# PKU-DAIR/Hetu-Galvatron

Measured on NVIDIA H100. Metric: tokens/sec Llama-3.2-1B-shaped ZeRO-2 training step at 1/2/4/8 H100 vs ref CPU, higher is better.
Workload: dtype bf16

## Files before the change

hetu-galvatron_b200/csrc/bg_gemm.cu:

```cuda
#include <stdlib.h>

#include "bg_ctx.cuh"

using namespace bg;

namespace {

constexpr int BLOCK_M = 128, BLOCK_N = 128, BLOCK_K = 64, WGMMA_K = 16;
constexpr int WIDE_N = 256;
constexpr int kABytes = BLOCK_M * BLOCK_K * 2;
constexpr int kStoreCols = 64;
constexpr int kStoreBytes = BLOCK_M * kStoreCols * 2;
constexpr int kEpiThreads = 256, kThreads = kEpiThreads + 32;
constexpr int kProducerWarp = kEpiThreads / 32;
constexpr int kWgOffset = 8192;
constexpr int kGroupM = 16;

template <int kBlockN>
struct Tile {
    static constexpr bool kWide = kBlockN == WIDE_N;
    static constexpr int kStages = kWide ? 4 : 5;
    static constexpr int kNumStoreBufs = kWide ? 1 : 2;
    static constexpr int kMaxRegs = kWide ? 168 : 136;
    static constexpr int kSlimCtas = kWide ? 2 : 3;
// ... 28 lines not shown
}
__device__ __forceinline__ void mbar_expect_tx(uint32_t bar, uint32_t bytes) {
    asm volatile("mbarrier.arrive.expect_tx.shared::cta.b64 _, [%0], %1;" ::"r"(bar), "r"(bytes) : "memory");
}
__device__ __forceinline__ void tma_load_2d(uint32_t dst, const CUtensorMap* map, uint32_t bar, int c0, int c1) {
    asm volatile("cp.async.bulk.tensor.2d.shared::cluster.global.mbarrier::complete_tx::bytes [%0], [%1, {%3, %4}], [%2];"
                 ::"r"(dst), "l"(map), "r"(bar), "r"(c0), "r"(c1) : "memory");
}
__device__ __forceinline__ void tma_store_2d(const CUtensorMap* map, uint32_t src, int c0, int c1) {
    asm volatile("cp.async.bulk.tensor.2d.global.shared::cta.bulk_group [%0, {%2, %3}], [%1];"
                 ::"l"(map), "r"(src), "r"(c0), "r"(c1) : "memory");
}
__device__ __forceinline__ void tma_store_commit() { asm volatile("cp.async.bulk.commit_group;" ::: "memory"); }
template <int N>
__device__ __forceinline__ void tma_store_wait_read() { asm volatile("cp.async.bulk.wait_group.read %0;" ::"n"(N) : "memory"); }
template <int N>
__device__ __forceinline__ void tma_store_wait_all() { asm volatile("cp.async.bulk.wait_group %0;" ::"n"(N) : "memory"); }
__device__ __forceinline__ void fence_proxy_async() { asm volatile("fence.proxy.async.shared::cta;" ::: "memory"); }
__device__ __forceinline__ void epi_bar_sync() { asm volatile("bar.sync 1, %0;" ::"n"(kEpiThreads) : "memory"); }
__device__ __forceinline__ bool elect_one() {
    uint32_t pred;
    asm volatile("{\n\t.reg .pred p;\n\telect.sync _|p, 0xffffffff;\n\tselp.u32 %0, 1, 0, p;\n\t}" : "=r"(pred));
    return pred != 0;
}

__device__ __forceinline__ void wgmma_fence() { asm volatile("wgmma.fence.sync.aligned;" ::: "memory"); }
__device__ __forceinline__ void wgmma_commit() { asm volatile("wgmma.commit_group.sync.aligned;" ::: "memory"); }
template <int N>
__device__ __forceinline__ void wgmma_wait() { asm volatile("wgmma.wait_group.sync.aligned %0;" ::"n"(N) : "memory"); }
template <int kNumAcc>
__device__ __forceinline__ void fence_acc(float* d) {
#pragma unroll
    for (int i = 0; i < kNumAcc; ++i) asm volatile("" : "+f"(d[i])::"memory");
}

template <int kTransA, int kTransB>
__device__ __forceinline__ void wgmma_m64n128(float* d, uint64_t desc_a, uint64_t desc_b, uint32_t accumulate) {
    asm volatile(
        "{\n\t.reg .pred p;\n\t"
        "setp.ne.b32 p, %66, 0;\n\t"
        "wgmma.mma_async.sync.aligned.m64n128k16.f32.bf16.bf16 "
        "{%0, %1, %2, %3, %4, %5, %6, %7, %8, %9, %10, %11, %12, %13, %14, %15, "
        "%16, %17, %18, %19, %20, %21, %22, %23, %24, %25, %26, %27, %28, %29, %30, %31, "
        "%32, %33, %34, %35, %36, %37, %38, %39, %40, %41, %42, %43, %44, %45, %46, %47, "
        "%48, %49, %50, %51, %52, %53, %54, %55, %56, %57, %58, %59, %60, %61, %62, %63}, "
        "%64, %65, p, 1, 1, %67, %68;\n\t}"
        : "+f"(d[0]), "+f"(d[1]), "+f"(d[2]), "+f"(d[3]), "+f"(d[4]), "+f"(d[5]), "+f"(d[6]), "+f"(d[7]),
          "+f"(d[8]), "+f"(d[9]), "+f"(d[10]), "+f"(d[11]), "+f"(d[12]), "+f"(d[13]), "+f"(d[14]), "+f"(d[15]),
          "+f"(d[16]), "+f"(d[17]), "+f"(d[18]), "+f"(d[19]), "+f"(d[20]), "+f"(d[21]), "+f"(d[22]), "+f"(d[23]),
          "+f"(d[24]), "+f"(d[25]), "+f"(d[26]), "+f"(d[27]), "+f"(d[28]), "+f"(d[29]), "+f"(d[30]), "+f"(d[31]),
          "+f"(d[32]), "+f"(d[33]), "+f"(d[34]), "+f"(d[35]), "+f"(d[36]), "+f"(d[37]), "+f"(d[38]), "+f"(d[39]),
          "+f"(d[40]), "+f"(d[41]), "+f"(d[42]), "+f"(d[43]), "+f"(d[44]), "+f"(d[45]), "+f"(d[46]), "+f"(d[47]),
          "+f"(d[48]), "+f"(d[49]), "+f"(d[50]), "+f"(d[51]), "+f"(d[52]), "+f"(d[53]), "+f"(d[54]), "+f"(d[55]),
          "+f"(d[56]), "+f"(d[57]), "+f"(d[58]), "+f"(d[59]), "+f"(d[60]), "+f"(d[61]), "+f"(d[62]), "+f"(d[63])
        : "l"(desc_a), "l"(desc_b), "r"(accumulate), "n"(kTransA), "n"(kTransB));
}

template <int kTransA, int kTransB>
__device__ __forceinline__ void wgmma_m64n256(float* d, uint64_t desc_a, uint64_t desc_b, uint32_t accumulate) {
    asm volatile(
        "{\n\t.reg .pred p;\n\t"
        "setp.ne.b32 p, %130, 0;\n\t"
        "wgmma.mma_async.sync.aligned.m64n256k16.f32.bf16.bf16 "
        "{%0, %1, %2, %3, %4, %5, %6, %7, %8, %9, %10, %11, %12, %13, %14, %15, "
        "%16, %17, %18, %19, %20, %21, %22, %23, %24, %25, %26, %27, %28, %29, %30, %31, "
        "%32, %33, %34, %35, %36, %37, %38, %39, %40, %41, %42, %43, %44, %45, %46, %47, "
// ... 9 lines not shown
          "+f"(d[24]), "+f"(d[25]), "+f"(d[26]), "+f"(d[27]), "+f"(d[28]), "+f"(d[29]), "+f"(d[30]), "+f"(d[31]),
          "+f"(d[32]), "+f"(d[33]), "+f"(d[34]), "+f"(d[35]), "+f"(d[36]), "+f"(d[37]), "+f"(d[38]), "+f"(d[39]),
          "+f"(d[40]), "+f"(d[41]), "+f"(d[42]), "+f"(d[43]), "+f"(d[44]), "+f"(d[45]), "+f"(d[46]), "+f"(d[47]),
          "+f"(d[48]), "+f"(d[49]), "+f"(d[50]), "+f"(d[51]), "+f"(d[52]), "+f"(d[53]), "+f"(d[54]), "+f"(d[55]),
          "+f"(d[56]), "+f"(d[57]), "+f"(d[58]), "+f"(d[59]), "+f"(d[60]), "+f"(d[61]), "+f"(d[62]), "+f"(d[63]),
          "+f"(d[64]), "+f"(d[65]), "+f"(d[66]), "+f"(d[67]), "+f"(d[68]), "+f"(d[69]), "+f"(d[70]), "+f"(d[71]),
          "+f"(d[72]), "+f"(d[73]), "+f"(d[74]), "+f"(d[75]), "+f"(d[76]), "+f"(d[77]), "+f"(d[78]), "+f"(d[79]),
          "+f"(d[80]), "+f"(d[81]), "+f"(d[82]), "+f"(d[83]), "+f"(d[84]), "+f"(d[85]), "+f"(d[86]), "+f"(d[87]),
          "+f"(d[88]), "+f"(d[89]), "+f"(d[90]), "+f"(d[91]), "+f"(d[92]), "+f"(d[93]), "+f"(d[94]), "+f"(d[95]),
          "+f"(d[96]), "+f"(d[97]), "+f"(d[98]), "+f"(d[99]), "+f"(d[100]), "+f"(d[101]), "+f"(d[102]), "+f"(d[103]),
          "+f"(d[104]), "+f"(d[105]), "+f"(d[106]), "+f"(d[107]), "+f"(d[108]), "+f"(d[109]), "+f"(d[110]), "+f"(d[111]),
          "+f"(d[112]), "+f"(d[113]), "+f"(d[114]), "+f"(d[115]), "+f"(d[116]), "+f"(d[117]), "+f"(d[118]), "+f"(d[119]),
          "+f"(d[120]), "+f"(d[121]), "+f"(d[122]), "+f"(d[123]), "+f"(d[124]), "+f"(d[125]), "+f"(d[126]), "+f"(d[127])
        : "l"(desc_a), "l"(desc_b), "r"(accumulate), "n"(kTransA), "n"(kTransB));
}

__device__ __forceinline__ uint64_t make_smem_desc(uint32_t smem_addr, uint32_t lbo_bytes, uint32_t sbo_bytes) {
    uint64_t d = 0;
    d |= (uint64_t)((smem_addr >> 4) & 0x3fff);
    d |= (uint64_t)((lbo_bytes >> 4) & 0x3fff) << 16;
    d |= (uint64_t)((sbo_bytes >> 4) & 0x3fff) << 32;
    d |= (uint64_t)1 << 62;
    return d;
}

struct TileCoord { int m, n; };
enum { kPlain = 0, kScatterMode = 1, kGatherMode = 2 };

template <int kMode>
struct FuseParams {};

template <>
struct FuseParams<kPlain> {
    int group_m;
};

__device__ __forceinline__ TileCoord tile_of_virtual(int t, int m_blocks, int n_blocks, int group_m) {
    const int per_group = group_m * n_blocks;
    const int g = t / per_group, first_m = g * group_m;
    const int rows = min(group_m, m_blocks - first_m);
    const int r = t - g * per_group;
    return {first_m + r % rows, r / rows};
}

template <>
struct FuseParams<kScatterMode> {
    CUtensorMap dst[BG_MAX_PEERS];
    uint32_t* flags[BG_MAX_PEERS];
    int p, me, rows_per_rank;
};

template <>
struct FuseParams<kGatherMode> {
    CUtensorMap a_local;
    const uint32_t* flags;
    uint32_t target;
    int p, me, blocks_per_rank;
    unsigned long long timeout_ns;
    int* err;
};

template <int kMode>
__device__ __forceinline__ int map_m(int mv, int m_blocks, const FuseParams<kMode>& fp) {
    if constexpr (kMode == kScatterMode) {
        int m = mv + ((fp.me + 1) % fp.p) * (fp.rows_per_rank / BLOCK_M);
        return m >= m_blocks ? m - m_blocks : m;
    } else if constexpr (kMode == kGatherMode) {
        const int c = mv / fp.p, k = mv - c * fp.p;
        int slot = fp.me + k; if (slot >= fp.p) slot -= fp.p;
        return slot * fp.blocks_per_rank + c;
    } else {
        return mv;
    }
}
template <int kMode>
__device__ __forceinline__ TileCoord tile_of(int t, int m_blocks, int n_blocks, const FuseParams<kMode>& fp) {
    int group_m = kGroupM;
    if constexpr (kMode == kPlain) group_m = fp.group_m;
    TileCoord tc = tile_of_virtual(t, m_blocks, n_blocks, group_m);
    tc.m = map_m<kMode>(tc.m, m_blocks, fp);
    return tc;
}

template <int kLayout, int kMode = kPlain, int kBlockN = BLOCK_N>
__global__ void __maxnreg__(Tile<kBlockN>::kMaxRegs) gemm_bf16_kernel(const __grid_constant__ CUtensorMap map_a,
                                                                const __grid_constant__ CUtensorMap map_b,
                                                                const __grid_constant__ CUtensorMap map_c,
                                                                const __nv_bfloat16* __restrict__ c_old, int M, int N, int K,
                                                                int accumulate,
                                                                const __grid_constant__ FuseParams<kMode> sp) {
    static_assert(kMode == kPlain || kBlockN == BLOCK_N, "the fused modes wait on peers: they keep the three-slim-CTA tile");
    constexpr bool kScatter = kMode == kScatterMode, kGather = kMode == kGatherMode;
    constexpr bool kAMn = kLayout == kNT, kBMn = kLayout != kTN;
    constexpr int kStages = Tile<kBlockN>::kStages, kStageBytes = Tile<kBlockN>::kStageBytes;
    constexpr int kNumStoreBufs = Tile<kBlockN>::kNumStoreBufs;
    extern __shared__ uint8_t smem_raw[];
    uint8_t* smem = reinterpret_cast<uint8_t*>((reinterpret_cast<uintptr_t>(smem_raw) + 1023) & ~uintptr_t(1023));
    uint8_t* smem_store = smem + kStages * kStageBytes;
    uint64_t* bars = reinterpret_cast<uint64_t*>(smem_store + kNumStoreBufs * kStoreBytes);
    uint64_t* full_bar = bars;
    uint64_t* empty_bar = bars + kStages;

    const int warp = threadIdx.x >> 5, lane = threadIdx.x & 31;
    const int m_blocks = (M + BLOCK_M - 1) / BLOCK_M, n_blocks = (N + kBlockN - 1) / kBlockN;
    const int num_tiles = m_blocks * n_blocks, k_blocks = (K + BLOCK_K - 1) / BLOCK_K;

    if constexpr (kScatter) {
        asm volatile("griddepcontrol.launch_dependents;" ::: "memory");
    }
    if (warp == kProducerWarp && lane == 0) {
        asm volatile("prefetch.tensormap [%0];" ::"l"(&map_a) : "memory");
        asm volatile("prefetch.tensormap [%0];" ::"l"(&map_b) : "memory");
        asm volatile("prefetch.tensormap [%0];" ::"l"(&map_c) : "memory");
        for (int i = 0; i < kStages; ++i) { mbar_init(smem_u32(full_bar + i), 1); mbar_init(smem_u32(empty_bar + i), kEpiThreads / 32); }
        asm volatile("fence.mbarrier_init.release.cluster;" ::: "memory");
    }
    __syncthreads();

    if (warp == kProducerWarp) {
        if (elect_one()) {
            int stage = 0; uint32_t phase = 0;
            for (int t = blockIdx.x; t < num_tiles; t += gridDim.x) {
                const TileCoord tc = tile_of<kMode>(t, m_blocks, n_blocks, sp);
                const CUtensorMap* amap = &map_a;
                int a_row = tc.m * BLOCK_M;
                if constexpr (kGather) {
                    const int slot = tc.m / sp.blocks_per_rank, c = tc.m - slot * sp.blocks_per_rank;
                    if (slot == sp.me) {
                        amap = &sp.a_local; a_row = c * BLOCK_M;
                    } else {
                        const uint32_t* f = sp.flags + slot * sp.blocks_per_rank + c;
                        unsigned long long t0 = 0; unsigned spins = 0;
                        while (true) {
                            uint32_t v;
                            asm volatile("ld.acquire.sys.global.u32 %0, [%1];" : "=r"(v) : "l"(f) : "memory");
                            if (v >= sp.target) break;
                            if ((++spins & 0x3ff) == 0) {
                                unsigned long long now = gtimer();
                                if (t0 == 0) t0 = now;
                                else if (now - t0 > sp.timeout_ns) {
                                    if (atomicCAS(sp.err + 1, 0, 4) == 0) { sp.err[2] = (int)blockIdx.x; sp.err[3] = tc.m; sp.err[4] = (int)v; sp.err[5] = (int)sp.target; sp.err[6] = slot; }
                                    *sp.err = BG_ETIMEOUT; __threadfence_system(); __trap();
                                }
                            }
                        }
                        asm volatile("fence.proxy.async.global;" ::: "memory");
                    }
// ... 2 lines not shown
                    mbar_wait(smem_u32(empty_bar + stage), phase ^ 1);
                    const uint32_t bar = smem_u32(full_bar + stage);
                    const uint32_t sa = smem_u32(smem + stage * kStageBytes), sb = sa + kABytes;
                    mbar_expect_tx(bar, kStageBytes);
                    if (kAMn) {
#pragma unroll
                        for (int j = 0; j < BLOCK_M / 64; ++j) tma_load_2d(sa + j * (BLOCK_K * 128), &map_a, bar, tc.m * BLOCK_M + j * 64, kb * BLOCK_K);
                    } else {
                        tma_load_2d(sa, amap, bar, kb * BLOCK_K, a_row);
                    }
                    if (kBMn) {
#pragma unroll
                        for (int j = 0; j < kBlockN / 64; ++j) tma_load_2d(sb + j * (BLOCK_K * 128), &map_b, bar, tc.n * kBlockN + j * 64, kb * BLOCK_K);
                    } else {
                        tma_load_2d(sb, &map_b, bar, kb * BLOCK_K, tc.n * kBlockN);
                    }
                    if (++stage == kStages) { stage = 0; phase ^= 1; }
                }
            }
        }
    } else {
        const int wg = warp >> 2;
        const int frag_row = wg * 64 + (warp & 3) * 16 + (lane >> 2);
        const int frag_col = (lane & 3) * 2;
        const bool issuer = threadIdx.x == 0;
        constexpr uint32_t a_lbo = kAMn ? BLOCK_K * 128 : 0, b_lbo = kBMn ? BLOCK_K * 128 : 0;
        constexpr uint32_t a_kstep = kAMn ? WGMMA_K * 128 : WGMMA_K * 2, b_kstep = kBMn ? WGMMA_K * 128 : WGMMA_K * 2;
        float acc[kBlockN / 2];
#pragma unroll
        for (int i = 0; i < kBlockN / 2; ++i) acc[i] = 0.f;
        int stage = 0; uint32_t phase = 0;
        int buf = 0;
        uint32_t* prev_flag = nullptr;
        for (int t = blockIdx.x; t < num_tiles; t += gridDim.x) {
            const TileCoord tc = tile_of<kMode>(t, m_blocks, n_blocks, sp);
            int prev_stage = 0;
            for (int kb = 0; kb < k_blocks; ++kb) {
                mbar_wait(smem_u32(full_bar + stage), phase);
                const uint32_t sa = smem_u32(smem + stage * kStageBytes) + wg * kWgOffset;
                const uint32_t sb = smem_u32(smem + stage * kStageBytes) + kABytes;
                wgmma_fence();
#pragma unroll
                for (int k = 0; k < BLOCK_K / WGMMA_K; ++k) {
                    const uint64_t da = make_smem_desc(sa + k * a_kstep, a_lbo, 1024);
                    const uint64_t db = make_smem_desc(sb + k * b_kstep, b_lbo, 1024);
                    if constexpr (kBlockN == WIDE_N) wgmma_m64n256<kAMn ? 1 : 0, kBMn ? 1 : 0>(acc, da, db, (kb | k) != 0);
                    else wgmma_m64n128<kAMn ? 1 : 0, kBMn ? 1 : 0>(acc, da, db, (kb | k) != 0);
                }
                wgmma_commit();
                wgmma_wait<1>();
                if (kb > 0 && lane == 0) mbar_arrive(smem_u32(empty_bar + prev_stage));
                prev_stage = stage;
                if (++stage == kStages) { stage = 0; phase ^= 1; }
            }
            wgmma_wait<0>();
            fence_acc<kBlockN / 2>(acc);
            if (lane == 0) mbar_arrive(smem_u32(empty_bar + prev_stage));
#pragma unroll
            for (int c = 0; c < kBlockN / kStoreCols; ++c) {
                const int n0 = tc.n * kBlockN + c * kStoreCols;
                if (n0 >= N) break;
                float* v = acc + c * (kStoreCols / 2);
                if (accumulate && Tile<kBlockN>::kWide) {
#pragma unroll
                    for (int h = 0; h < 2; ++h) {
                        const int grow = tc.m * BLOCK_M + frag_row + 8 * h;
                        if (grow < M) {
                            const uint32_t* src = reinterpret_cast<const uint32_t*>(c_old + (long long)grow * N + n0 + frag_col);
#pragma unroll
                            for (int j = 0; j < 8; ++j) {
                                if (n0 + j * 8 < N) {
                                    const float2 o = bf2_to_f2(src[j * 4]);
                                    v[j * 4 + 2 * h] += o.x;
                                    v[j * 4 + 2 * h + 1] += o.y;
                                }
                            }
                        }
                    }
                } else if (accumulate) {
#pragma unroll
                    for (int h = 0; h < 2; ++h) {
                        const long long grow = (long long)tc.m * BLOCK_M + frag_row + 8 * h;
                        if (grow < M) {
#pragma unroll
                            for (int j = 0; j < 8; ++j) {
                                if (n0 + j * 8 < N) {
                                    const float2 o = bf2_to_f2(*reinterpret_cast<const uint32_t*>(c_old + grow * N + n0 + j * 8 + frag_col));
                                    v[j * 4 + 2 * h] += o.x;
                                    v[j * 4 + 2 * h + 1] += o.y;
                                }
                            }
                        }
                    }
                }
                if (issuer) tma_store_wait_read<kNumStoreBufs - 1>();
                epi_bar_sync();
                uint8_t* sbuf = smem_store + buf * kStoreBytes;
                if constexpr (Tile<kBlockN>::kWide) {
                    uint32_t srow = smem_u32(sbuf) + frag_row * 128 + ((frag_row & 7) << 4) + frag_col * 2;
                    asm volatile("" : "+r"(srow));
#pragma unroll
                    for (int h = 0; h < 2; ++h) {
#pragma unroll
                        for (int j = 0; j < 8; ++j)
                            asm volatile("st.shared.u32 [%0], %1;" ::"r"((srow + h * 1024) ^ (j << 4)),
                                         "r"(f2_to_bf2(v[j * 4 + 2 * h], v[j * 4 + 2 * h + 1])) : "memory");
                    }
                } else {
#pragma unroll
                    for (int h = 0; h < 2; ++h) {
                        const int row = frag_row + 8 * h;
#pragma unroll
                        for (int j = 0; j < 8; ++j)
                            *reinterpret_cast<uint32_t*>(sbuf + row * 128 + ((j ^ (row & 7)) << 4) + frag_col * 2) =
                                f2_to_bf2(v[j * 4 + 2 * h], v[j * 4 + 2 * h + 1]);
                    }
                }
                fence_proxy_async();
                epi_bar_sync();
                if (issuer) {
                    if constexpr (kScatter) {
                        const int row0 = tc.m * BLOCK_M, owner = row0 / sp.rows_per_rank;
                        tma_store_2d(&sp.dst[owner], smem_u32(sbuf), n0, sp.me * sp.rows_per_rank + (row0 - owner * sp.rows_per_rank));
                    } else {
                        tma_store_2d(&map_c, smem_u32(sbuf), n0, tc.m * BLOCK_M);
                    }
                    tma_store_commit();
                }
                if constexpr (kNumStoreBufs > 1) buf ^= 1;
            }
            if constexpr (kScatter) {
                if (issuer) {
                    if (prev_flag != nullptr) {
                        asm volatile("cp.async.bulk.wait_group %0;" ::"n"(kBlockN / kStoreCols) : "memory");
                        __threadfence_system();
                        asm volatile("red.release.sys.global.add.u32 [%0], 1;" ::"l"(prev_flag) : "memory");
                    }
                    const int row0 = tc.m * BLOCK_M, owner = row0 / sp.rows_per_rank;
                    prev_flag = sp.flags[owner] + ((row0 - owner * sp.rows_per_rank) / BLOCK_M) * n_blocks + tc.n;
                }
            }
        }
        if (issuer) {
            tma_store_wait_all<0>();
            if constexpr (kScatter) {
                if (prev_flag != nullptr) {
                    __threadfence_system();
                    asm volatile("red.release.sys.global.add.u32 [%0], 1;" ::"l"(prev_flag) : "memory");
                }
            }
        }
    }
}

typedef CUresult (*EncodeTiledFn)(CUtensorMap*, CUtensorMapDataType, cuuint32_t, void*, const cuuint64_t*, const cuuint64_t*,
                                  const cuuint32_t*, const cuuint32_t*, CUtensorMapInterleave, CUtensorMapSwizzle,
                                  CUtensorMapL2promotion, CUtensorMapFloatOOBfill);

EncodeTiledFn encode_fn() {
    static EncodeTiledFn fn = nullptr;
    static std::once_flag once;
    std::call_once(once, [] {
        void* p = nullptr;
        cudaDriverEntryPointQueryResult q;
        if (cudaGetDriverEntryPoint("cuTensorMapEncodeTiled", &p, cudaEnableDefault, &q) == cudaSuccess && q == cudaDriverEntryPointSuccess)
            fn = (EncodeTiledFn)p;
    });
    return fn;
}

int make_map(CUtensorMap* map, const void* ptr, long long rows, long long cols, int box_cols, int box_rows) {
    EncodeTiledFn fn = encode_fn();
    if (!fn) return fail(BG_ECUDA, "cuTensorMapEncodeTiled entry point not available");
    cuuint64_t dims[2] = {(cuuint64_t)cols, (cuuint64_t)rows};
    cuuint64_t strides[1] = {(cuuint64_t)cols * 2};
    cuuint32_t box[2] = {(cuuint32_t)box_cols, (cuuint32_t)box_rows};
    cuuint32_t estr[2] = {1, 1};
    CUresult r = fn(map, CU_TENSOR_MAP_DATA_TYPE_BFLOAT16, 2, const_cast<void*>(ptr), dims, strides, box, estr,
                    CU_TENSOR_MAP_INTERLEAVE_NONE, CU_TENSOR_MAP_SWIZZLE_128B, CU_TENSOR_MAP_L2_PROMOTION_L2_256B,
                    CU_TENSOR_MAP_FLOAT_OOB_FILL_NONE);
    if (r == CUDA_ERROR_INVALID_CONTEXT) {
        cudaFree(0);
        r = fn(map, CU_TENSOR_MAP_DATA_TYPE_BFLOAT16, 2, const_cast<void*>(ptr), dims, strides, box, estr,
               CU_TENSOR_MAP_INTERLEAVE_NONE, CU_TENSOR_MAP_SWIZZLE_128B, CU_TENSOR_MAP_L2_PROMOTION_L2_256B,
               CU_TENSOR_MAP_FLOAT_OOB_FILL_NONE);
    }
    if (r != CUDA_SUCCESS) return fail(BG_ECUDA, "cuTensorMapEncodeTiled failed (%d) rows=%lld cols=%lld", (int)r, rows, cols);
    return BG_OK;
}

int g_num_sms = 0;

}

int bg_preload_gemm();

static int gemm_setup() {
    if (g_num_sms == 0) {
        int dev = 0;
        BG_CUDA(cudaGetDevice(&dev));
        int sms = 0;
        BG_CUDA(cudaDeviceGetAttribute(&sms, cudaDevAttrMultiProcessorCount, dev));
#define BG_SMEM(K, W) BG_CUDA(cudaFuncSetAttribute(K, cudaFuncAttributeMaxDynamicSharedMemorySize, Tile<W>::kSmemBytes))
        BG_SMEM(gemm_bf16_kernel<kTN>, BLOCK_N); BG_SMEM(gemm_bf16_kernel<kNN>, BLOCK_N); BG_SMEM(gemm_bf16_kernel<kNT>, BLOCK_N);
        BG_SMEM((gemm_bf16_kernel<kTN, kPlain, WIDE_N>), WIDE_N); BG_SMEM((gemm_bf16_kernel<kNN, kPlain, WIDE_N>), WIDE_N);
        BG_SMEM((gemm_bf16_kernel<kNT, kPlain, WIDE_N>), WIDE_N);
        BG_SMEM((gemm_bf16_kernel<kTN, kScatterMode>), BLOCK_N); BG_SMEM((gemm_bf16_kernel<kNN, kScatterMode>), BLOCK_N);
        BG_SMEM((gemm_bf16_kernel<kNT, kScatterMode>), BLOCK_N);
        BG_SMEM((gemm_bf16_kernel<kTN, kGatherMode>), BLOCK_N); BG_SMEM((gemm_bf16_kernel<kNN, kGatherMode>), BLOCK_N);
#undef BG_SMEM
        g_num_sms = sms;
    }
    return BG_OK;
}



static int make_ab_maps(CUtensorMap* ma, CUtensorMap* mb, const void* a, const void* b, long long m, long long n, long long k, int layout,
                        int block_n = BLOCK_N) {
    int rc = layout == kNT ? make_map(ma, a, k, m, 64, BLOCK_K) : make_map(ma, a, m, k, BLOCK_K, BLOCK_M);
    if (rc) return rc;
    return layout == kTN ? make_map(mb, b, n, k, BLOCK_K, block_n) : make_map(mb, b, k, n, 64, BLOCK_K);
}

static int gemm_launch(const void* a, const void* b, void* c, const void* addend, long long m, long long n, long long k, int layout, void* stream);

extern "C" int bg_gemm_bf16(const void* a, const void* b, void* c, long long m, long long n, long long k, int layout,
                            int accumulate, void* stream) {
    return gemm_launch(a, b, c, accumulate ? c : nullptr, m, n, k, layout, stream);
}

extern "C" int bg_gemm_bf16_add(const void* a, const void* b, void* c, const void* addend, long long m, long long n, long long k,
                                int layout, void* stream) {
    if (addend == nullptr || (uintptr_t)addend % 16) return fail(BG_EINVAL, "bg_gemm_bf16_add: addend must be a 16-B aligned [M][N] bf16 tensor");
    return gemm_launch(a, b, c, addend, m, n, k, layout, stream);
}

template <int kBlockN>
static int plain_launch(const void* a, const void* b, void* c, const void* addend, long long m, long long n, long long k, int layout, void* stream);

static int gemm_launch(const void* a, const void* b, void* c, const void* addend, long long m, long long n, long long k, int layout, void* stream) {
    if (layout < 0 || layout > 2) return fail(BG_EINVAL, "bg_gemm_bf16: layout %d", layout);
    if (m <= 0 || n <= 0 || k <= 0 || m % 8 || n % 8 || k % 8)
        return fail(BG_EINVAL, "bg_gemm_bf16: m,n,k (%lld,%lld,%lld) must be positive multiples of 8", m, n, k);
    if (((uintptr_t)a | (uintptr_t)b | (uintptr_t)c) % 16) return fail(BG_EINVAL, "bg_gemm_bf16: pointers must be 16-B aligned");
    return n > BLOCK_N ? plain_launch<WIDE_N>(a, b, c, addend, m, n, k, layout, stream)
                       : plain_launch<BLOCK_N>(a, b, c, addend, m, n, k, layout, stream);
}

template <int kBlockN>
static int plain_launch(const void* a, const void* b, void* c, const void* addend, long long m, long long n, long long k, int layout, void* stream) {
    CUtensorMap ma, mb, mc;
    int rc = make_ab_maps(&ma, &mb, a, b, m, n, k, layout, kBlockN);
    if (rc) return rc;
    rc = make_map(&mc, c, m, n, kStoreCols, BLOCK_M);
    if (rc) return rc;
    rc = gemm_setup();
    if (rc) return rc;
    const long long n_blocks = (n + kBlockN - 1) / kBlockN, tiles = ((m + BLOCK_M - 1) / BLOCK_M) * n_blocks;
    const int grid = (int)(tiles < g_num_sms ? tiles : g_num_sms);
    cudaStream_t st = (cudaStream_t)stream;
    const __nv_bfloat16* c_old = (const __nv_bfloat16*)addend;
    const int accumulate = addend != nullptr;
    constexpr int smem = Tile<kBlockN>::kSmemBytes;
    FuseParams<kPlain> plain;
    plain.group_m = n_blocks <= 16 ? 4 : 16;
    if (layout == kTN) gemm_bf16_kernel<kTN, kPlain, kBlockN><<<grid, kThreads, smem, st>>>(ma, mb, mc, c_old, (int)m, (int)n, (int)k, accumulate, plain);
    else if (layout == kNN) gemm_bf16_kernel<kNN, kPlain, kBlockN><<<grid, kThreads, smem, st>>>(ma, mb, mc, c_old, (int)m, (int)n, (int)k, accumulate, plain);
    else gemm_bf16_kernel<kNT, kPlain, kBlockN><<<grid, kThreads, smem, st>>>(ma, mb, mc, c_old, (int)m, (int)n, (int)k, accumulate, plain);
    BG_CHECK_LAUNCH();
    return BG_OK;
}

namespace {

struct Bcast {
    char* out[BG_MAX_PEERS];
    char* mc;
    int on;
};

__device__ __forceinline__ void mm_st_16g(void* mc, const uint4& v) {
    asm volatile("multimem.st.relaxed.sys.global.v4.f32 [%0], {%1,%2,%3,%4};" ::"l"(mc), "f"(__uint_as_float(v.x)),
                 "f"(__uint_as_float(v.y)), "f"(__uint_as_float(v.z)), "f"(__uint_as_float(v.w)) : "memory");
}

__global__ void __launch_bounds__(128, 8) tile_reduce_kernel(const __nv_bfloat16* __restrict__ partial, uint32_t* __restrict__ flags,
                                                          __nv_bfloat16* __restrict__ out, int p, int me, int rows_per_rank, int N,
                                                          int n_blocks, int local_tiles, const __grid_constant__ Bcast bc,
                                                          unsigned long long timeout_ns, int* err) {
    for (int lt = blockIdx.x; lt < local_tiles; lt += gridDim.x) {
        if (threadIdx.x == 0) {
            unsigned long long t0 = 0;
            unsigned spins = 0;
            while (true) {
                uint32_t v;
                asm volatile("ld.acquire.sys.global.u32 %0, [%1];" : "=r"(v) : "l"(flags + lt) : "memory");
                if (v >= (uint32_t)p) break;
                if ((++spins & 0x3ff) == 0) {
                    unsigned long long now = gtimer();
                    if (t0 == 0) t0 = now;
                    else if (now - t0 > timeout_ns / 2) {
// ... 45 lines not shown
        if (threadIdx.x == 0) flags[lt] = 0;
    }
    asm volatile("griddepcontrol.wait;" ::: "memory");
}

}

int bg_gemm_scatter_maps(FusedGemmMaps* maps, const void* a, const void* b, long long m, long long n, long long k, int layout, int p,
                         void* const* partial_ptrs) {
    int rc = make_ab_maps(&maps->a, &maps->b, a, b, m, n, k, layout);
    if (rc) return rc;
    for (int i = 0; i < BG_MAX_PEERS; ++i) {
        if (i < p) { rc = make_map(&maps->peer[i], partial_ptrs[i], m, n, kStoreCols, BLOCK_M); if (rc) return rc; }
        else maps->peer[i] = maps->peer[0];
    }
    return gemm_setup();
}

int bg_gemm_scatter_launch(const FusedGemmMaps& maps, long long m, long long n, long long k, int layout, int p, int me,
                           void* const* partial_ptrs, uint32_t* const* flag_ptrs, void* out, void* const* bcast_ptrs, char* bcast_mc,
                           unsigned long long timeout_ns, int* err_dev, cudaStream_t st) {
    const int rows_per_rank = (int)(m / p);
    FuseParams<kScatterMode> sp;
    sp.p = p; sp.me = me; sp.rows_per_rank = rows_per_rank;
    for (int i = 0; i < BG_MAX_PEERS; ++i) {
        sp.flags[i] = i < p ? flag_ptrs[i] : nullptr;
        sp.dst[i] = maps.peer[i];
    }
    const int m_blocks = (int)((m + BLOCK_M - 1) / BLOCK_M), n_blocks = (int)((n + BLOCK_N - 1) / BLOCK_N);
    const long long tiles = (long long)m_blocks * n_blocks;
    const int grid = (int)(tiles < g_num_sms ? tiles : g_num_sms);
    const int local_tiles = (rows_per_rank / BLOCK_M) * n_blocks;
    const CUtensorMap& mc_unused = sp.dst[0];
    if (layout == kTN) gemm_bf16_kernel<kTN, kScatterMode><<<grid, kThreads, Tile<BLOCK_N>::kSmemBytes, st>>>(maps.a, maps.b, mc_unused, nullptr, (int)m, (int)n, (int)k, 0, sp);
    else if (layout == kNN) gemm_bf16_kernel<kNN, kScatterMode><<<grid, kThreads, Tile<BLOCK_N>::kSmemBytes, st>>>(maps.a, maps.b, mc_unused, nullptr, (int)m, (int)n, (int)k, 0, sp);
    else gemm_bf16_kernel<kNT, kScatterMode><<<grid, kThreads, Tile<BLOCK_N>::kSmemBytes, st>>>(maps.a, maps.b, mc_unused, nullptr, (int)m, (int)n, (int)k, 0, sp);
    BG_CHECK_LAUNCH();
    const int rgrid = local_tiles < g_num_sms ? local_tiles : g_num_sms;
    Bcast bc = {};
    if (bcast_ptrs != nullptr) {
        bc.on = 1; bc.mc = bcast_mc;
        for (int i = 0; i < p; ++i) bc.out[i] = (char*)bcast_ptrs[i];
    }
    cudaLaunchConfig_t cfg = {};
    cfg.gridDim = dim3((unsigned)rgrid); cfg.blockDim = dim3(128);
    cfg.dynamicSmemBytes = 0; cfg.stream = st;
    cudaLaunchAttribute attr[1];
    attr[0].id = cudaLaunchAttributeProgrammaticStreamSerialization;
    attr[0].val.programmaticStreamSerializationAllowed = 1;
    static const bool no_pdl = getenv("HGB_NO_PDL") != nullptr;
    cfg.attrs = attr; cfg.numAttrs = no_pdl ? 0 : 1;
    BG_CUDA(cudaLaunchKernelEx(&cfg, tile_reduce_kernel, (const __nv_bfloat16*)partial_ptrs[me], (uint32_t*)flag_ptrs[me],
                               (__nv_bfloat16*)out, p, me, rows_per_rank, (int)n, n_blocks, local_tiles, bc, timeout_ns, err_dev));
    bg::g_launches.fetch_add(1, std::memory_order_relaxed);
    return BG_OK;
}

int bg_gemm_gather_maps(FusedGemmMaps* maps, const void* a_local, const void* a_staged, const void* b, void* c, long long m, long long n,
                        long long k, int layout, int p) {
    int rc = make_ab_maps(&maps->a, &maps->b, a_staged, b, m, n, k, layout);
    if (rc) return rc;
    rc = make_map(&maps->c, c, m, n, kStoreCols, BLOCK_M);
    if (rc) return rc;
    rc = make_map(&maps->peer[0], a_local, m / p, k, BLOCK_K, BLOCK_M);
    if (rc) return rc;
    return gemm_setup();
}

int bg_gemm_gather_launch(const FusedGemmMaps& maps, long long m, long long n, long long k, int layout, int p, int me,
                          const uint32_t* flags, uint32_t target, unsigned long long timeout_ns, int* err_dev, cudaStream_t st) {
    FuseParams<kGatherMode> gp;
    gp.a_local = maps.peer[0];
    gp.flags = flags; gp.target = target; gp.p = p; gp.me = me; gp.blocks_per_rank = (int)(m / p / BLOCK_M);
    gp.timeout_ns = timeout_ns; gp.err = err_dev;
    const long long tiles = (m / BLOCK_M) * ((n + BLOCK_N - 1) / BLOCK_N);
    const int grid = (int)(tiles < g_num_sms ? tiles : g_num_sms);
    if (layout == kTN) gemm_bf16_kernel<kTN, kGatherMode><<<grid, kThreads, Tile<BLOCK_N>::kSmemBytes, st>>>(maps.a, maps.b, maps.c, nullptr, (int)m, (int)n, (int)k, 0, gp);
    else gemm_bf16_kernel<kNN, kGatherMode><<<grid, kThreads, Tile<BLOCK_N>::kSmemBytes, st>>>(maps.a, maps.b, maps.c, nullptr, (int)m, (int)n, (int)k, 0, gp);
    BG_CHECK_LAUNCH();
    return BG_OK;
}

int bg_preload_gemm() {
    int rc = gemm_setup();
    if (rc) return rc;
    cudaFuncAttributes attr;
    BG_CUDA(cudaFuncGetAttributes(&attr, reinterpret_cast<const void*>(&tile_reduce_kernel)));
    return BG_OK;
}
```

Baseline: 55150.

## TMA-prefetch addend into borrowed pipeline stage for wide-tile GEMM epilogue

For the 256-wide tile, the epilogue now loads the addend matrix C with TMA into shared memory instead of reading it with scattered global loads. The first chunk goes into the store buffer early in the mainloop, and the remaining chunks go into the last pipeline stage, which is held back until its stores have drained. The whole 128x256 tile is then staged in shared memory and written with one batch of TMA stores. Separately, the launcher now picks the narrow 128-column tile when wave quantization makes it markedly better-balanced. The cost is more complex barrier and stage-borrowing logic, and one pipeline stage is held longer per tile, which may reduce producer lookahead.

```diff
diff --git a/hetu-galvatron_b200/csrc/bg_gemm.cu b/hetu-galvatron_b200/csrc/bg_gemm.cu
--- a/hetu-galvatron_b200/csrc/bg_gemm.cu
+++ b/hetu-galvatron_b200/csrc/bg_gemm.cu
@@ -159,6 +159,7 @@
 
 template <>
 struct FuseParams<kPlain> {
+    CUtensorMap c_in;
     int group_m;
 };
 
@@ -218,6 +219,7 @@
                                                                 const __grid_constant__ FuseParams<kMode> sp) {
     static_assert(kMode == kPlain || kBlockN == BLOCK_N, "the fused modes wait on peers: they keep the three-slim-CTA tile");
     constexpr bool kScatter = kMode == kScatterMode, kGather = kMode == kGatherMode;
+    constexpr bool kWide = Tile<kBlockN>::kWide;
     constexpr bool kAMn = kLayout == kNT, kBMn = kLayout != kTN;
     constexpr int kStages = Tile<kBlockN>::kStages, kStageBytes = Tile<kBlockN>::kStageBytes;
     constexpr int kNumStoreBufs = Tile<kBlockN>::kNumStoreBufs;
@@ -227,6 +229,7 @@
     uint64_t* bars = reinterpret_cast<uint64_t*>(smem_store + kNumStoreBufs * kStoreBytes);
     uint64_t* full_bar = bars;
     uint64_t* empty_bar = bars + kStages;
+    uint64_t* c_bar = bars + 2 * kStages;
 
     const int warp = threadIdx.x >> 5, lane = threadIdx.x & 31;
     const int m_blocks = (M + BLOCK_M - 1) / BLOCK_M, n_blocks = (N + kBlockN - 1) / kBlockN;
@@ -240,6 +243,10 @@
         asm volatile("prefetch.tensormap [%0];" ::"l"(&map_b) : "memory");
         asm volatile("prefetch.tensormap [%0];" ::"l"(&map_c) : "memory");
         for (int i = 0; i < kStages; ++i) { mbar_init(smem_u32(full_bar + i), 1); mbar_init(smem_u32(empty_bar + i), kEpiThreads / 32); }
+        if constexpr (kWide) {
+            if (accumulate) asm volatile("prefetch.tensormap [%0];" ::"l"(&sp.c_in) : "memory");
+            mbar_init(smem_u32(c_bar), 1); mbar_init(smem_u32(c_bar + 1), 1);
+        }
         asm volatile("fence.mbarrier_init.release.cluster;" ::: "memory");
     }
     __syncthreads();
@@ -308,6 +315,8 @@
         int stage = 0; uint32_t phase = 0;
         int buf = 0;
         uint32_t* prev_flag = nullptr;
+        int borrowed = -1;
+        uint32_t c_phase = 0;
         for (int t = blockIdx.x; t < num_tiles; t += gridDim.x) {
             const TileCoord tc = tile_of<kMode>(t, m_blocks, n_blocks, sp);
             int prev_stage = 0;
@@ -326,63 +335,93 @@
                 wgmma_commit();
                 wgmma_wait<1>();
                 if (kb > 0 && lane == 0) mbar_arrive(smem_u32(empty_bar + prev_stage));
+                if constexpr (kWide) {
+                    if (kb == 0 && issuer) {
+                        if (borrowed >= 0) {
+                            tma_store_wait_read<0>();
+                            mbar_arrive(smem_u32(empty_bar + borrowed));
+                        }
+                        if (accumulate) {
+                            mbar_expect_tx(smem_u32(c_bar), kStoreBytes);
+                            tma_load_2d(smem_u32(smem_store), &sp.c_in, smem_u32(c_bar), tc.n * kBlockN, tc.m * BLOCK_M);
+                        }
+                    }
+                }
                 prev_stage = stage;
                 if (++stage == kStages) { stage = 0; phase ^= 1; }
             }
             wgmma_wait<0>();
             fence_acc<kBlockN / 2>(acc);
-            if (lane == 0) mbar_arrive(smem_u32(empty_bar + prev_stage));
-#pragma unroll
-            for (int c = 0; c < kBlockN / kStoreCols; ++c) {
-                const int n0 = tc.n * kBlockN + c * kStoreCols;
-                if (n0 >= N) break;
-                float* v = acc + c * (kStoreCols / 2);
-                if (accumulate && Tile<kBlockN>::kWide) {
+            if constexpr (kWide) {
+                if (lane == 0 && !issuer) mbar_arrive(smem_u32(empty_bar + prev_stage));
+                borrowed = prev_stage;
+                const int n_first = tc.n * kBlockN, m_first = tc.m * BLOCK_M;
+                const int n_chunks = min(kBlockN / kStoreCols, (N - n_first + kStoreCols - 1) / kStoreCols);
+                const uint32_t s_borrowed = smem_u32(smem + borrowed * kStageBytes);
+                epi_bar_sync();
+                if (accumulate && issuer) {
+                    mbar_expect_tx(smem_u32(c_bar + 1), (n_chunks - 1) * kStoreBytes);
+                    for (int c = 1; c < n_chunks; ++c)
+                        tma_load_2d(s_borrowed + (c - 1) * kStoreBytes, &sp.c_in, smem_u32(c_bar + 1), n_first + c * kStoreCols, m_first);
+                }
+                uint32_t srow = frag_row * 128 + ((frag_row & 7) << 4) + frag_col * 2;
+                asm volatile("" : "+r"(srow));
+#pragma unroll
+                for (int c = 0; c < kBlockN / kStoreCols; ++c) {
+                    if (c >= n_chunks) break;
+                    if (accumulate && c < 2) mbar_wait(smem_u32(c_bar + c), c_phase);
+                    const uint32_t sbox = c == 0 ? smem_u32(smem_store) : s_borrowed + (c - 1) * kStoreBytes;
+                    float* v = acc + c * (kStoreCols / 2);
 #pragma unroll
                     for (int h = 0; h < 2; ++h) {
-                        const int grow = tc.m * BLOCK_M + frag_row + 8 * h;
-                        if (grow < M) {
-                            const uint32_t* src = reinterpret_cast<const uint32_t*>(c_old + (long long)grow * N + n0 + frag_col);
-#pragma unroll
-                            for (int j = 0; j < 8; ++j) {
-                                if (n0 + j * 8 < N) {
-                                    const float2 o = bf2_to_f2(src[j * 4]);
-                                    v[j * 4 + 2 * h] += o.x;
-                                    v[j * 4 + 2 * h + 1] += o.y;
+#pragma unroll
+                        for (int j = 0; j < 8; ++j) {
+                            const uint32_t addr = sbox + ((srow + h * 1024) ^ (j << 4));
+                            if (accumulate) {
+                                uint32_t o;
+                                asm volatile("ld.shared.u32 %0, [%1];" : "=r"(o) : "r"(addr) : "memory");
+                                const float2 f = bf2_to_f2(o);
+                                v[j * 4 + 2 * h] += f.x;
+                                v[j * 4 + 2 * h + 1] += f.y;
+                            }
+                            asm volatile("st.shared.u32 [%0], %1;" ::"r"(addr), "r"(f2_to_bf2(v[j * 4 + 2 * h], v[j * 4 + 2 * h + 1])) : "memory");
+                        }
+                    }
+                }
+                if (accumulate) c_phase ^= 1;
+                fence_proxy_async();
+                epi_bar_sync();
+                if (issuer) {
+                    for (int c = 0; c < n_chunks; ++c)
+                        tma_store_2d(&map_c, c == 0 ? smem_u32(smem_store) : s_borrowed + (c - 1) * kStoreBytes, n_first + c * kStoreCols, m_first);
+                    tma_store_commit();
+                }
+            } else {
+                if (lane == 0) mbar_arrive(smem_u32(empty_bar + prev_stage));
+#pragma unroll
+                for (int c = 0; c < kBlockN / kStoreCols; ++c) {
+                    const int n0 = tc.n * kBlockN + c * kStoreCols;
+                    if (n0 >= N) break;
+                    float* v = acc + c * (kStoreCols / 2);
+                    if (accumulate) {
+#pragma unroll
+                        for (int h = 0; h < 2; ++h) {
+                            const long long grow = (long long)tc.m * BLOCK_M + frag_row + 8 * h;
+                            if (grow < M) {
+#pragma unroll
+                                for (int j = 0; j < 8; ++j) {
+                                    if (n0 + j * 8 < N) {
+                                        const float2 o = bf2_to_f2(*reinterpret_cast<const uint32_t*>(c_old + grow * N + n0 + j * 8 + frag_col));
+                                        v[j * 4 + 2 * h] += o.x;
+                                        v[j * 4 + 2 * h + 1] += o.y;
+                                    }
                                 }
                             }
                         }
                     }
-                } else if (accumulate) {
-#pragma unroll
-                    for (int h = 0; h < 2; ++h) {
-                        const long long grow = (long long)tc.m * BLOCK_M + frag_row + 8 * h;
-                        if (grow < M) {
-#pragma unroll
-                            for (int j = 0; j < 8; ++j) {
-                                if (n0 + j * 8 < N) {
-                                    const float2 o = bf2_to_f2(*reinterpret_cast<const uint32_t*>(c_old + grow * N + n0 + j * 8 + frag_col));
-                                    v[j * 4 + 2 * h] += o.x;
-                                    v[j * 4 + 2 * h + 1] += o.y;
-                                }
-                            }
-                        }
-                    }
-                }
-                if (issuer) tma_store_wait_read<kNumStoreBufs - 1>();
-                epi_bar_sync();
-                uint8_t* sbuf = smem_store + buf * kStoreBytes;
-                if constexpr (Tile<kBlockN>::kWide) {
-                    uint32_t srow = smem_u32(sbuf) + frag_row * 128 + ((frag_row & 7) << 4) + frag_col * 2;
-                    asm volatile("" : "+r"(srow));
-#pragma unroll
-                    for (int h = 0; h < 2; ++h) {
-#pragma unroll
-                        for (int j = 0; j < 8; ++j)
-                            asm volatile("st.shared.u32 [%0], %1;" ::"r"((srow + h * 1024) ^ (j << 4)),
-                                         "r"(f2_to_bf2(v[j * 4 + 2 * h], v[j * 4 + 2 * h + 1])) : "memory");
-                    }
-                } else {
+                    if (issuer) tma_store_wait_read<kNumStoreBufs - 1>();
+                    epi_bar_sync();
+                    uint8_t* sbuf = smem_store + buf * kStoreBytes;
 #pragma unroll
                     for (int h = 0; h < 2; ++h) {
                         const int row = frag_row + 8 * h;
@@ -391,34 +430,35 @@
                             *reinterpret_cast<uint32_t*>(sbuf + row * 128 + ((j ^ (row & 7)) << 4) + frag_col * 2) =
                                 f2_to_bf2(v[j * 4 + 2 * h], v[j * 4 + 2 * h + 1]);
                     }
-                }
-                fence_proxy_async();
-                epi_bar_sync();
-                if (issuer) {
-                    if constexpr (kScatter) {
+                    fence_proxy_async();
+                    epi_bar_sync();
+                    if (issuer) {
+                        if constexpr (kScatter) {
+                            const int row0 = tc.m * BLOCK_M, owner = row0 / sp.rows_per_rank;
+                            tma_store_2d(&sp.dst[owner], smem_u32(sbuf), n0, sp.me * sp.rows_per_rank + (row0 - owner * sp.rows_per_rank));
+                        } else {
+                            tma_store_2d(&map_c, smem_u32(sbuf), n0, tc.m * BLOCK_M);
+                        }
+                        tma_store_commit();
+                    }
+                    if constexpr (kNumStoreBufs > 1) buf ^= 1;
+                }
+                if constexpr (kScatter) {
+                    if (issuer) {
+                        if (prev_flag != nullptr) {
+                            asm volatile("cp.async.bulk.wait_group %0;" ::"n"(kBlockN / kStoreCols) : "memory");
+                            __threadfence_system();
+                            asm volatile("red.release.sys.global.add.u32 [%0], 1;" ::"l"(prev_flag) : "memory");
+                        }
                         const int row0 = tc.m * BLOCK_M, owner = row0 / sp.rows_per_rank;
-                        tma_store_2d(&sp.dst[owner], smem_u32(sbuf), n0, sp.me * sp.rows_per_rank + (row0 - owner * sp.rows_per_rank));
-                    } else {
-                        tma_store_2d(&map_c, smem_u32(sbuf), n0, tc.m * BLOCK_M);
-                    }
-                    tma_store_commit();
-                }
-                if constexpr (kNumStoreBufs > 1) buf ^= 1;
-            }
-            if constexpr (kScatter) {
-                if (issuer) {
-                    if (prev_flag != nullptr) {
-                        asm volatile("cp.async.bulk.wait_group %0;" ::"n"(kBlockN / kStoreCols) : "memory");
-                        __threadfence_system();
-                        asm volatile("red.release.sys.global.add.u32 [%0], 1;" ::"l"(prev_flag) : "memory");
-                    }
-                    const int row0 = tc.m * BLOCK_M, owner = row0 / sp.rows_per_rank;
-                    prev_flag = sp.flags[owner] + ((row0 - owner * sp.rows_per_rank) / BLOCK_M) * n_blocks + tc.n;
+                        prev_flag = sp.flags[owner] + ((row0 - owner * sp.rows_per_rank) / BLOCK_M) * n_blocks + tc.n;
+                    }
                 }
             }
         }
         if (issuer) {
             tma_store_wait_all<0>();
+            if constexpr (kWide) mbar_arrive(smem_u32(empty_bar + borrowed));
             if constexpr (kScatter) {
                 if (prev_flag != nullptr) {
                     __threadfence_system();
@@ -520,8 +560,14 @@
     if (m <= 0 || n <= 0 || k <= 0 || m % 8 || n % 8 || k % 8)
         return fail(BG_EINVAL, "bg_gemm_bf16: m,n,k (%lld,%lld,%lld) must be positive multiples of 8", m, n, k);
     if (((uintptr_t)a | (uintptr_t)b | (uintptr_t)c) % 16) return fail(BG_EINVAL, "bg_gemm_bf16: pointers must be 16-B aligned");
-    return n > BLOCK_N ? plain_launch<WIDE_N>(a, b, c, addend, m, n, k, layout, stream)
-                       : plain_launch<BLOCK_N>(a, b, c, addend, m, n, k, layout, stream);
+    int rc = gemm_setup();
+    if (rc) return rc;
+    if (n <= BLOCK_N) return plain_launch<BLOCK_N>(a, b, c, addend, m, n, k, layout, stream);
+    const long long m_blocks = (m + BLOCK_M - 1) / BLOCK_M, wide_tiles = m_blocks * ((n + WIDE_N - 1) / WIDE_N);
+    const auto busy = [&](long long tiles) { return (double)tiles / (double)((tiles + g_num_sms - 1) / g_num_sms * g_num_sms); };
+    const bool narrow = wide_tiles >= g_num_sms && busy(m_blocks * ((n + BLOCK_N - 1) / BLOCK_N)) > 1.3 * busy(wide_tiles);
+    return narrow ? plain_launch<BLOCK_N>(a, b, c, addend, m, n, k, layout, stream)
+                  : plain_launch<WIDE_N>(a, b, c, addend, m, n, k, layout, stream);
 }
 
 template <int kBlockN>
@@ -539,8 +585,12 @@
     const __nv_bfloat16* c_old = (const __nv_bfloat16*)addend;
     const int accumulate = addend != nullptr;
     constexpr int smem = Tile<kBlockN>::kSmemBytes;
-    FuseParams<kPlain> plain;
+    FuseParams<kPlain> plain = {};
     plain.group_m = n_blocks <= 16 ? 4 : 16;
+    if (kBlockN == WIDE_N && accumulate) {
+        rc = make_map(&plain.c_in, addend, m, n, kStoreCols, BLOCK_M);
+        if (rc) return rc;
+    }
     if (layout == kTN) gemm_bf16_kernel<kTN, kPlain, kBlockN><<<grid, kThreads, smem, st>>>(ma, mb, mc, c_old, (int)m, (int)n, (int)k, accumulate, plain);
     else if (layout == kNN) gemm_bf16_kernel<kNN, kPlain, kBlockN><<<grid, kThreads, smem, st>>>(ma, mb, mc, c_old, (int)m, (int)n, (int)k, accumulate, plain);
     else gemm_bf16_kernel<kNT, kPlain, kBlockN><<<grid, kThreads, smem, st>>>(ma, mb, mc, c_old, (int)m, (int)n, (int)k, accumulate, plain);
```

Result: faster. 55890 (median of 6 runs) (+1.3%).

## Prefetch GEMM addend into registers ahead of epilogue and pick tile width by wave fill

Applied to the files above, without the earlier changes.

The runtime accumulate flag becomes a template parameter. The old C addend is now loaded into registers before the final wgmma wait, and the next 64-column chunk is prefetched while the current one is being stored, so global-load latency overlaps the MMA tail and the shared-memory stores. A wave-fill heuristic can now choose 128-wide tiles over 256-wide tiles when the wide tiling would leave SMs idle. The kb loop is also unrolled by two in the non-addend path. These changes add template instantiations and register pressure in the epilogue.

```diff
diff --git a/hetu-galvatron_b200/csrc/bg_gemm.cu b/hetu-galvatron_b200/csrc/bg_gemm.cu
--- a/hetu-galvatron_b200/csrc/bg_gemm.cu
+++ b/hetu-galvatron_b200/csrc/bg_gemm.cu
@@ -84,6 +84,18 @@
 __device__ __forceinline__ void fence_acc(float* d) {
 #pragma unroll
     for (int i = 0; i < kNumAcc; ++i) asm volatile("" : "+f"(d[i])::"memory");
+}
+
+__device__ __forceinline__ void load_c_chunk(uint32_t (&r)[16], const __nv_bfloat16* c, int row, int col, int M, int N) {
+    const __nv_bfloat16* p = c + (long long)row * N + col;
+#pragma unroll
+    for (int h = 0; h < 2; ++h) {
+#pragma unroll
+        for (int j = 0; j < 8; ++j)
+            asm volatile("{\n\t.reg .pred p;\n\tsetp.ne.b32 p, %2, 0;\n\tmov.b32 %0, 0;\n\t@p ld.global.b32 %0, [%1];\n\t}"
+                         : "=r"(r[j * 2 + h])
+                         : "l"(p + (long long)h * 8 * N + j * 8), "r"((int)(row + 8 * h < M && col + j * 8 < N)));
+    }
 }
 
 template <int kTransA, int kTransB>
@@ -209,14 +221,14 @@
     return tc;
 }
 
-template <int kLayout, int kMode = kPlain, int kBlockN = BLOCK_N>
+template <int kLayout, int kMode = kPlain, int kBlockN = BLOCK_N, bool kReadC = false>
 __global__ void __maxnreg__(Tile<kBlockN>::kMaxRegs) gemm_bf16_kernel(const __grid_constant__ CUtensorMap map_a,
                                                                 const __grid_constant__ CUtensorMap map_b,
                                                                 const __grid_constant__ CUtensorMap map_c,
                                                                 const __nv_bfloat16* __restrict__ c_old, int M, int N, int K,
-                                                                int accumulate,
                                                                 const __grid_constant__ FuseParams<kMode> sp) {
     static_assert(kMode == kPlain || kBlockN == BLOCK_N, "the fused modes wait on peers: they keep the three-slim-CTA tile");
+    static_assert(kMode == kPlain || !kReadC, "the fused modes store their product as it is");
     constexpr bool kScatter = kMode == kScatterMode, kGather = kMode == kGatherMode;
     constexpr bool kAMn = kLayout == kNT, kBMn = kLayout != kTN;
     constexpr int kStages = Tile<kBlockN>::kStages, kStageBytes = Tile<kBlockN>::kStageBytes;
@@ -311,6 +323,7 @@
         for (int t = blockIdx.x; t < num_tiles; t += gridDim.x) {
             const TileCoord tc = tile_of<kMode>(t, m_blocks, n_blocks, sp);
             int prev_stage = 0;
+#pragma unroll (kReadC ? 1 : 2)
             for (int kb = 0; kb < k_blocks; ++kb) {
                 mbar_wait(smem_u32(full_bar + stage), phase);
                 const uint32_t sa = smem_u32(smem + stage * kStageBytes) + wg * kWgOffset;
@@ -329,6 +342,9 @@
                 prev_stage = stage;
                 if (++stage == kStages) { stage = 0; phase ^= 1; }
             }
+            uint32_t c_pre[16];
+            const bool read_c = kReadC && c_old != nullptr;
+            if (read_c) load_c_chunk(c_pre, c_old, tc.m * BLOCK_M + frag_row, tc.n * kBlockN + frag_col, M, N);
             wgmma_wait<0>();
             fence_acc<kBlockN / 2>(acc);
             if (lane == 0) mbar_arrive(smem_u32(empty_bar + prev_stage));
@@ -337,41 +353,20 @@
                 const int n0 = tc.n * kBlockN + c * kStoreCols;
                 if (n0 >= N) break;
                 float* v = acc + c * (kStoreCols / 2);
-                if (accumulate && Tile<kBlockN>::kWide) {
-#pragma unroll
-                    for (int h = 0; h < 2; ++h) {
-                        const int grow = tc.m * BLOCK_M + frag_row + 8 * h;
-                        if (grow < M) {
-                            const uint32_t* src = reinterpret_cast<const uint32_t*>(c_old + (long long)grow * N + n0 + frag_col);
-#pragma unroll
-                            for (int j = 0; j < 8; ++j) {
-                                if (n0 + j * 8 < N) {
-                                    const float2 o = bf2_to_f2(src[j * 4]);
-                                    v[j * 4 + 2 * h] += o.x;
-                                    v[j * 4 + 2 * h + 1] += o.y;
-                                }
-                            }
-                        }
-                    }
-                } else if (accumulate) {
-#pragma unroll
-                    for (int h = 0; h < 2; ++h) {
-                        const long long grow = (long long)tc.m * BLOCK_M + frag_row + 8 * h;
-                        if (grow < M) {
-#pragma unroll
-                            for (int j = 0; j < 8; ++j) {
-                                if (n0 + j * 8 < N) {
-                                    const float2 o = bf2_to_f2(*reinterpret_cast<const uint32_t*>(c_old + grow * N + n0 + j * 8 + frag_col));
-                                    v[j * 4 + 2 * h] += o.x;
-                                    v[j * 4 + 2 * h + 1] += o.y;
-                                }
-                            }
-                        }
-                    }
-                }
                 if (issuer) tma_store_wait_read<kNumStoreBufs - 1>();
                 epi_bar_sync();
                 uint8_t* sbuf = smem_store + buf * kStoreBytes;
+                if (read_c) {
+#pragma unroll
+                    for (int j = 0; j < 8; ++j) {
+#pragma unroll
+                        for (int h = 0; h < 2; ++h) {
+                            const float2 o = bf2_to_f2(c_pre[j * 2 + h]);
+                            v[j * 4 + 2 * h] += o.x;
+                            v[j * 4 + 2 * h + 1] += o.y;
+                        }
+                    }
+                }
                 if constexpr (Tile<kBlockN>::kWide) {
                     uint32_t srow = smem_u32(sbuf) + frag_row * 128 + ((frag_row & 7) << 4) + frag_col * 2;
                     asm volatile("" : "+r"(srow));
@@ -379,7 +374,7 @@
                     for (int h = 0; h < 2; ++h) {
 #pragma unroll
                         for (int j = 0; j < 8; ++j)
-                            asm volatile("st.shared.u32 [%0], %1;" ::"r"((srow + h * 1024) ^ (j << 4)),
+                            asm volatile("st.shared.u32 [%0], %1;" ::"r"((srow ^ (j << 4)) + h * 1024),
                                          "r"(f2_to_bf2(v[j * 4 + 2 * h], v[j * 4 + 2 * h + 1])) : "memory");
                     }
                 } else {
@@ -391,6 +386,10 @@
                             *reinterpret_cast<uint32_t*>(sbuf + row * 128 + ((j ^ (row & 7)) << 4) + frag_col * 2) =
                                 f2_to_bf2(v[j * 4 + 2 * h], v[j * 4 + 2 * h + 1]);
                     }
+                }
+                if (read_c) {
+                    if (c + 1 < kBlockN / kStoreCols)
+                        load_c_chunk(c_pre, c_old, tc.m * BLOCK_M + frag_row, n0 + kStoreCols + frag_col, M, N);
                 }
                 fence_proxy_async();
                 epi_bar_sync();
@@ -481,6 +480,10 @@
         BG_SMEM(gemm_bf16_kernel<kTN>, BLOCK_N); BG_SMEM(gemm_bf16_kernel<kNN>, BLOCK_N); BG_SMEM(gemm_bf16_kernel<kNT>, BLOCK_N);
         BG_SMEM((gemm_bf16_kernel<kTN, kPlain, WIDE_N>), WIDE_N); BG_SMEM((gemm_bf16_kernel<kNN, kPlain, WIDE_N>), WIDE_N);
         BG_SMEM((gemm_bf16_kernel<kNT, kPlain, WIDE_N>), WIDE_N);
+        BG_SMEM((gemm_bf16_kernel<kTN, kPlain, BLOCK_N, true>), BLOCK_N); BG_SMEM((gemm_bf16_kernel<kNN, kPlain, BLOCK_N, true>), BLOCK_N);
+        BG_SMEM((gemm_bf16_kernel<kNT, kPlain, BLOCK_N, true>), BLOCK_N);
+        BG_SMEM((gemm_bf16_kernel<kTN, kPlain, WIDE_N, true>), WIDE_N); BG_SMEM((gemm_bf16_kernel<kNN, kPlain, WIDE_N, true>), WIDE_N);
+        BG_SMEM((gemm_bf16_kernel<kNT, kPlain, WIDE_N, true>), WIDE_N);
         BG_SMEM((gemm_bf16_kernel<kTN, kScatterMode>), BLOCK_N); BG_SMEM((gemm_bf16_kernel<kNN, kScatterMode>), BLOCK_N);
         BG_SMEM((gemm_bf16_kernel<kNT, kScatterMode>), BLOCK_N);
         BG_SMEM((gemm_bf16_kernel<kTN, kGatherMode>), BLOCK_N); BG_SMEM((gemm_bf16_kernel<kNN, kGatherMode>), BLOCK_N);
@@ -515,13 +518,25 @@
 template <int kBlockN>
 static int plain_launch(const void* a, const void* b, void* c, const void* addend, long long m, long long n, long long k, int layout, void* stream);
 
+static bool wide_tiles(long long m, long long n, int sms) {
+    if (n <= BLOCK_N) return false;
+    const long long m_blocks = (m + BLOCK_M - 1) / BLOCK_M;
+    auto fill = [&](int block_n) {
+        const long long tiles = m_blocks * ((n + block_n - 1) / block_n), waves = (tiles + sms - 1) / sms;
+        return (double)tiles / (double)(waves * sms);
+    };
+    return !(fill(WIDE_N) < 0.75 && fill(BLOCK_N) >= 0.9);
+}
+
 static int gemm_launch(const void* a, const void* b, void* c, const void* addend, long long m, long long n, long long k, int layout, void* stream) {
     if (layout < 0 || layout > 2) return fail(BG_EINVAL, "bg_gemm_bf16: layout %d", layout);
     if (m <= 0 || n <= 0 || k <= 0 || m % 8 || n % 8 || k % 8)
         return fail(BG_EINVAL, "bg_gemm_bf16: m,n,k (%lld,%lld,%lld) must be positive multiples of 8", m, n, k);
     if (((uintptr_t)a | (uintptr_t)b | (uintptr_t)c) % 16) return fail(BG_EINVAL, "bg_gemm_bf16: pointers must be 16-B aligned");
-    return n > BLOCK_N ? plain_launch<WIDE_N>(a, b, c, addend, m, n, k, layout, stream)
-                       : plain_launch<BLOCK_N>(a, b, c, addend, m, n, k, layout, stream);
+    int rc = gemm_setup();
+    if (rc) return rc;
+    return wide_tiles(m, n, g_num_sms) ? plain_launch<WIDE_N>(a, b, c, addend, m, n, k, layout, stream)
+                                       : plain_launch<BLOCK_N>(a, b, c, addend, m, n, k, layout, stream);
 }
 
 template <int kBlockN>
@@ -537,13 +552,16 @@
     const int grid = (int)(tiles < g_num_sms ? tiles : g_num_sms);
     cudaStream_t st = (cudaStream_t)stream;
     const __nv_bfloat16* c_old = (const __nv_bfloat16*)addend;
-    const int accumulate = addend != nullptr;
     constexpr int smem = Tile<kBlockN>::kSmemBytes;
     FuseParams<kPlain> plain;
     plain.group_m = n_blocks <= 16 ? 4 : 16;
-    if (layout == kTN) gemm_bf16_kernel<kTN, kPlain, kBlockN><<<grid, kThreads, smem, st>>>(ma, mb, mc, c_old, (int)m, (int)n, (int)k, accumulate, plain);
-    else if (layout == kNN) gemm_bf16_kernel<kNN, kPlain, kBlockN><<<grid, kThreads, smem, st>>>(ma, mb, mc, c_old, (int)m, (int)n, (int)k, accumulate, plain);
-    else gemm_bf16_kernel<kNT, kPlain, kBlockN><<<grid, kThreads, smem, st>>>(ma, mb, mc, c_old, (int)m, (int)n, (int)k, accumulate, plain);
+#define BG_PLAIN(L, C) gemm_bf16_kernel<L, kPlain, kBlockN, C><<<grid, kThreads, smem, st>>>(ma, mb, mc, c_old, (int)m, (int)n, (int)k, plain)
+    if (c_old != nullptr) {
+        if (layout == kTN) BG_PLAIN(kTN, true); else if (layout == kNN) BG_PLAIN(kNN, true); else BG_PLAIN(kNT, true);
+    } else {
+        if (layout == kTN) BG_PLAIN(kTN, false); else if (layout == kNN) BG_PLAIN(kNN, false); else BG_PLAIN(kNT, false);
+    }
+#undef BG_PLAIN
     BG_CHECK_LAUNCH();
     return BG_OK;
 }
@@ -655,9 +673,9 @@
     const int grid = (int)(tiles < g_num_sms ? tiles : g_num_sms);
     const int local_tiles = (rows_per_rank / BLOCK_M) * n_blocks;
     const CUtensorMap& mc_unused = sp.dst[0];
-    if (layout == kTN) gemm_bf16_kernel<kTN, kScatterMode><<<grid, kThreads, Tile<BLOCK_N>::kSmemBytes, st>>>(maps.a, maps.b, mc_unused, nullptr, (int)m, (int)n, (int)k, 0, sp);
-    else if (layout == kNN) gemm_bf16_kernel<kNN, kScatterMode><<<grid, kThreads, Tile<BLOCK_N>::kSmemBytes, st>>>(maps.a, maps.b, mc_unused, nullptr, (int)m, (int)n, (int)k, 0, sp);
-    else gemm_bf16_kernel<kNT, kScatterMode><<<grid, kThreads, Tile<BLOCK_N>::kSmemBytes, st>>>(maps.a, maps.b, mc_unused, nullptr, (int)m, (int)n, (int)k, 0, sp);
+    if (layout == kTN) gemm_bf16_kernel<kTN, kScatterMode><<<grid, kThreads, Tile<BLOCK_N>::kSmemBytes, st>>>(maps.a, maps.b, mc_unused, nullptr, (int)m, (int)n, (int)k, sp);
+    else if (layout == kNN) gemm_bf16_kernel<kNN, kScatterMode><<<grid, kThreads, Tile<BLOCK_N>::kSmemBytes, st>>>(maps.a, maps.b, mc_unused, nullptr, (int)m, (int)n, (int)k, sp);
+    else gemm_bf16_kernel<kNT, kScatterMode><<<grid, kThreads, Tile<BLOCK_N>::kSmemBytes, st>>>(maps.a, maps.b, mc_unused, nullptr, (int)m, (int)n, (int)k, sp);
     BG_CHECK_LAUNCH();
     const int rgrid = local_tiles < g_num_sms ? local_tiles : g_num_sms;
     Bcast bc = {};
@@ -698,8 +716,8 @@
     gp.timeout_ns = timeout_ns; gp.err = err_dev;
     const long long tiles = (m / BLOCK_M) * ((n + BLOCK_N - 1) / BLOCK_N);
     const int grid = (int)(tiles < g_num_sms ? tiles : g_num_sms);
-    if (layout == kTN) gemm_bf16_kernel<kTN, kGatherMode><<<grid, kThreads, Tile<BLOCK_N>::kSmemBytes, st>>>(maps.a, maps.b, maps.c, nullptr, (int)m, (int)n, (int)k, 0, gp);
-    else gemm_bf16_kernel<kNN, kGatherMode><<<grid, kThreads, Tile<BLOCK_N>::kSmemBytes, st>>>(maps.a, maps.b, maps.c, nullptr, (int)m, (int)n, (int)k, 0, gp);
+    if (layout == kTN) gemm_bf16_kernel<kTN, kGatherMode><<<grid, kThreads, Tile<BLOCK_N>::kSmemBytes, st>>>(maps.a, maps.b, maps.c, nullptr, (int)m, (int)n, (int)k, gp);
+    else gemm_bf16_kernel<kNN, kGatherMode><<<grid, kThreads, Tile<BLOCK_N>::kSmemBytes, st>>>(maps.a, maps.b, maps.c, nullptr, (int)m, (int)n, (int)k, gp);
     BG_CHECK_LAUNCH();
     return BG_OK;
 }
```

Measured after the change: 54510 before, 55300 after, median of 6. +1.4%, better.
